# duyhominhnguyen/conan-fgw

Measured on AMD Instinct MI355X. Metric: molecules/s (K=5 conformers), higher is better.
Workload: dtype f32

## Files before the change

conan-fgw_amd/csrc/fgw_common.h:

```cpp
#pragma once
#include "common.h"

#ifdef CONAN_FGW_PROFILE
static __device__ long long g_fgw_prof[32];
#define FGW_PROF_ACCESSOR(name)                                                          \
    extern "C" int name(long long *out, int reset) {                                     \
        if (out && hipMemcpyFromSymbol(out, HIP_SYMBOL(g_fgw_prof), sizeof(long long) * 32) != hipSuccess) return -2; \
        if (reset) { long long z[32] = {0}; if (hipMemcpyToSymbol(HIP_SYMBOL(g_fgw_prof), z, sizeof(z)) != hipSuccess) return -2; } \
        return 0;                                                                        \
    }
static __device__ long long g_fgw_trace[2 + 6 * 8192];
#define FGW_PROF_TRACE_ACCESSOR(name)                                                    \
    extern "C" int name(long long *out, int reset) {                                     \
        if (out && hipMemcpyFromSymbol(out, HIP_SYMBOL(g_fgw_trace), sizeof(long long) * (2 + 6 * 8192)) != hipSuccess) return -2; \
        if (reset) { long long z[2] = {0, 0}; if (hipMemcpyToSymbol(HIP_SYMBOL(g_fgw_trace), z, sizeof(z)) != hipSuccess) return -2; } \
        return 0;                                                                        \
    }
#define FGW_PROF_TRACE(tag)                                                              \
    do {                                                                                 \
        if (threadIdx.x == 0) {                                                          \
            const unsigned long long i_ = atomicAdd(reinterpret_cast<unsigned long long *>(&g_fgw_trace[0]), 1ull); \
            if (i_ < 8192) {                                                             \
                long long *r_ = &g_fgw_trace[2 + 6 * i_];                                \
                r_[0] = (long long)blockIdx.x; r_[1] = (long long)(tag);                 \
// ... 214 lines not shown
                for (int u = 0; u < 4; ++u) a[u] = (double)xr[kb + u];
                if (WT) {
                    const TW *wr = W + (size_t)jc * pW + kb;
#pragma unroll
                    for (int u = 0; u < 4; ++u) b[u] = (double)wr[u];
                } else {
#pragma unroll
                    for (int u = 0; u < 4; ++u) b[u] = (double)W[(size_t)(kb + u) * pW + jc];
                }
            } else {
#pragma unroll
                for (int u = 0; u < 4; ++u) {
                    const int k = kb + u, kc = k < Kd ? k : Kd - 1;
                    const double av = (double)xr[kc], bv = (double)(WT ? W[(size_t)jc * pW + kc] : W[(size_t)kc * pW + jc]);
                    a[u] = k < Kd ? av : 0.0; b[u] = k < Kd ? bv : 0.0;
                }
            }
            acc = __builtin_amdgcn_mfma_f64_16x16x4f64(ra ? a[0] : 0.0, cb ? b[0] : 0.0, acc, 0, 0, 0);
            acc2 = __builtin_amdgcn_mfma_f64_16x16x4f64(ra ? a[1] : 0.0, cb ? b[1] : 0.0, acc2, 0, 0, 0);
            acc = __builtin_amdgcn_mfma_f64_16x16x4f64(ra ? a[2] : 0.0, cb ? b[2] : 0.0, acc, 0, 0, 0);
            acc2 = __builtin_amdgcn_mfma_f64_16x16x4f64(ra ? a[3] : 0.0, cb ? b[3] : 0.0, acc2, 0, 0, 0);
        }
#pragma unroll
        for (int q = 0; q < 4; ++q) {
            const int i = i0 + lk + 4 * q;
            if (i < M && cb) st(i, jb, acc[q] + acc2[q]);
        }
    }
}

template <int NT>
__device__ __forceinline__ void fgw_order_by_size(const FgwAdj &adj, int B, int K, int tid) {
    static_assert(NT >= 256, "one thread per size bin");
    __shared__ unsigned char nsz[4096];
    __shared__ int hist[256], base[256];
    if (B > 4096) return;
    for (int t = tid; t < 256; t += NT) hist[t] = 0;
    __syncthreads();
    for (int m = tid; m < B; m += NT) {
        const int n = min(max(adj.gptr[m * K + 1] - adj.gptr[m * K], 0), 255);
        nsz[m] = (unsigned char)n;
        atomicAdd(&hist[n], 1);
    }
    __syncthreads();
    if (tid == 0) {
        int run = 0;
        for (int v = 255; v >= 0; --v) { base[v] = run; run += hist[v]; }
    }
    __syncthreads();
    if (tid < 256 && hist[tid] > 0) {
        int pos = base[tid];
        for (int m = 0; m < B; ++m)
            if (nsz[m] == (unsigned char)tid) adj.order[pos++] = m;
    }
}

#ifndef CONAN_FGW_KT
#define CONAN_FGW_KT 2
#endif
template <int NW, bool WT, typename TX, typename TW, class FS, int KT = CONAN_FGW_KT>
__device__ __forceinline__ void mm_f64_glb22(int M, int Nn, int Kd, const TX *__restrict__ X, int pX, const TW *__restrict__ W, int pW, FS st,
                                             const int tid = threadIdx.x) {
    const int lane = tid & 63, wave = __builtin_amdgcn_readfirstlane(tid >> 6);
    const int Mq = (M + 15) >> 4, Nq = (Nn + 15) >> 4;
    const int li = lane & 15, lk = lane >> 4;
    const int Mb = Mq >> 1, Nb = Nq >> 1;
    const int nblk = Mb * Nb, nblk_used = (nblk / NW) * NW;
    auto load_a = [&](const TX *xr, int kb, int k0, double (&a)[KT]) {
        if (k0 + 4 * KT <= Kd) {
#pragma unroll
            for (int u = 0; u < KT; ++u) a[u] = (double)xr[kb + u];
        } else {
#pragma unroll
            for (int u = 0; u < KT; ++u) { const int k = kb + u; const double v = (double)xr[k < Kd ? k : Kd - 1]; a[u] = k < Kd ? v : 0.0; }
        }
    };
    auto load_b = [&](int jc, int kb, int k0, double (&b)[KT]) {
        if (k0 + 4 * KT <= Kd) {
#pragma unroll
            for (int u = 0; u < KT; ++u) b[u] = (double)(WT ? W[(size_t)jc * pW + kb + u] : W[(size_t)(kb + u) * pW + jc]);
        } else {
#pragma unroll
            for (int u = 0; u < KT; ++u) {
                const int k = kb + u, kc = k < Kd ? k : Kd - 1;
                const double v = (double)(WT ? W[(size_t)jc * pW + kc] : W[(size_t)kc * pW + jc]);
// ... 616 lines not shown
```

conan-fgw_amd/csrc/fgw_small.hip:

```cpp
#include "fgw_common.h"

#ifdef CONAN_FGW_PROFILE
FGW_PROF_ACCESSOR(conan_debug_fgw_prof)
FGW_PROF_TRACE_ACCESSOR(conan_debug_fgw_trace)
#endif

namespace {

constexpr int SK_SCRATCH_DOUBLES = 3 * 256 + 2 * 64;

template <int R, bool KL, bool SECOND = false>
__global__ void __launch_bounds__(FGW_THREADS, (SECOND || R > 9) ? 1 : 3) k_fgw_coupling_small(
    const float *__restrict__ Ys, const float *__restrict__ Cs, const float *__restrict__ ps, const float *__restrict__ pb,
    FgwDims D, conan_fgw_params prm, int outer, int y_zero, const double *__restrict__ Cw, const double *__restrict__ Yw,
    const int *__restrict__ active, float *__restrict__ Tw, int *__restrict__ info, fgw_part_t *__restrict__ Ypart,
    fgw_part_t *__restrict__ Cpart, const double *__restrict__ zvec, const double *__restrict__ yvec, const int *__restrict__ only, FgwAdj adj) {
    extern __shared__ __attribute__((aligned(16))) char smem[];
    auto solve = [&](const int cid) {
    const int b = cid / D.K, s = cid % D.K;
    if (!fgw_active(active, D.B, b, outer)) return;
    const int N = D.N, P = D.P, d = D.d;
    const int NN = N * N, NP = N * P;
    const int tid = threadIdx.x, lane = tid & 63, w = __builtin_amdgcn_readfirstlane(tid >> 6);
    const bool lane_ok = lane < N;
    FGW_PROF_DECL;

    double *Al = reinterpret_cast<double *>(smem);
    double *Gl = Al + NP;
    double *C1l = Gl + NP;
    double *Bl = C1l + NP;
    double *pq = Bl + NP;
    double *red = pq + 128;
    float *t_dummy = reinterpret_cast<float *>(red + 7);
    double *vec4 = red + 8;
    const bool alias = (size_t)NP >= SK_SCRATCH_DOUBLES;
    double *own = vec4 + 256;
    double *bufC = alias ? Al : own;
    double *bufK = bufC + 256;
    double *bufR = bufK + 256;
    double *fcp = bufR + 256;
    double *gcp = fcp + 64;
    float *Tl = reinterpret_cast<float *>(own + (alias ? 0 : SK_SCRATCH_DOUBLES));
// ... 11 lines not shown
    float *Tg = Tw + ((size_t)b * D.K + s) * NN;
    const double alpha = (double)prm.alpha, inv_eps = 1.0 / (double)prm.epsilon;

    constexpr int EPT = (16 * R * R + FGW_THREADS - 1) / FGW_THREADS;
    double c1v[EPT];
    float c2v[EPT], tv[EPT];
    const bool warm = outer > 0 && prm.warmstart;
#pragma unroll
    for (int u = 0; u < EPT; ++u) {
        const int t = tid + u * FGW_THREADS, tc = t < NN ? t : NN - 1;
        c1v[u] = C1[tc]; c2v[u] = C2[tc]; tv[u] = warm ? Tg[tc] : 0.f;
    }
    const double p_own = tid < N ? (pb ? (double)pb[(size_t)b * N + tid] : 1.0 / (double)N) : 1.0;
    const double q_own = tid < N ? (ps ? (double)ps[((size_t)b * D.K + s) * N + tid] : 1.0 / (double)N) : 1.0;
    double vec_own;
    {
        const int v = tid >> 6, i = tid & 63;
        const double *src = (v == 0 || v == 2) ? yvec + (size_t)b * 2 * N + (v == 0 ? N : 0) : zvec + ((size_t)b * D.K + s) * 2 * N + (v == 1 ? N : 0);
        vec_own = src[i < N ? i : N - 1];
        vec_own = i < N ? vec_own : 0.0;
    }
    const bool stage_yz = yz_lds && !y_zero;
    if (stage_yz) {
        const int Nd = N * d;
        for (int t0 = tid; t0 < Nd; t0 += 4 * FGW_THREADS) {
            double yv[4]; float zv[4];
#pragma unroll
            for (int u = 0; u < 4; ++u) { const int t = t0 + u * FGW_THREADS, tc = t < Nd ? t : Nd - 1; yv[u] = Y[tc]; zv[u] = Z[tc]; }
#pragma unroll
            for (int u = 0; u < 4; ++u) { const int t = t0 + u * FGW_THREADS; if (t < Nd) { Yl[t] = yv[u]; Zl[t] = zv[u]; } }
        }
    }
    if (tid < 64) { pq[tid] = p_own; pq[64 + tid] = q_own; }
    const bool massless = __syncthreads_or(tid < N && (p_own <= 0.0 || q_own <= 0.0)) != 0;
    vec4[tid] = vec_own;
#pragma unroll
    for (int u = 0; u < EPT; ++u) {
        const int t = tid + u * FGW_THREADS;
        if (t < NN) { const int i = t / N, j = t - i * N; C2l[i * P + j] = c2v[u]; if (!stage_yz) C1l[i * P + j] = c1v[u]; }
    }
    __syncthreads();
    FGW_PROF(0);
    const double qj = pq[64 + lane];
    const double pi_l = pq[lane];
#pragma unroll
    for (int u = 0; u < EPT; ++u) {
        const int t = tid + u * FGW_THREADS;
        if (t < NN) { const int i = t / N, j = t - i * N; Tl[i * P + j] = warm ? tv[u] : (float)(pq[i] * pq[64 + j]); }
    }
    const double *r1v = vec4, *r2v = vec4 + 64, *y2v = vec4 + 128, *z2v = vec4 + 192;
    double *Dl = stage_yz ? C1l : Al;
    if (!y_zero) {
        if (stage_yz)
            mm_lds<FGW_WAVES, true>(N, N, d, Yl, d, Zl, d, [&](int i, int j, double v) { Dl[i * P + j] = v; }, border_prepare(N, N));
        else
            mm_f64(N, N, d, [&](int i, int k) { return Y[(size_t)i * d + k]; }, [&](int k, int j) { return (double)Z[(size_t)j * d + k]; },
                   [&](int i, int j, double v) { Dl[i * P + j] = v; });
    }
    __syncthreads();
    FGW_PROF(1);
#pragma unroll
    for (int u = 0; u < EPT; ++u) {
        const int t = tid + u * FGW_THREADS;
        if (t < NN) {
            const int i = t / N, j = t - i * N;
            double m = -2.0 * (y_zero ? 0.0 : Dl[i * P + j]); m += y2v[i]; m += z2v[j];
            m = m > 0.0 ? m : 0.0;
// ... 138 lines not shown
                         xs[192 + lane] * exp_lse(m3 - M);
                    u_l = lane_ok ? loga - (log_acc(sm) + M) : 0.0;
                }
                uc[lane] = u_l;
                if (ii % 10 == 0) {
                    double cs = 0.0;
#pragma unroll
                    for (int r = 0; r < R; ++r) cs += exp_acc(mrA(r) + uc[w + 4 * r] + v_l);
                    __syncthreads();
                    xs[w * 64 + lane] = cs;
                    __syncthreads();
                    cs = ((xs[lane] + xs[64 + lane]) + xs[128 + lane]) + xs[192 + lane];
                    double df = lane_ok ? cs - qj : 0.0;
                    df = wave_sum_d(df * df);
                    if (sqrt(df) < (double)prm.stop_thr) { ++ii; break; }
                }
            }
#pragma unroll
            for (int r = 0; r < R; ++r) kA[r] = exp_acc(mrA(r) + uc[w + 4 * r] + v_l);
        }
        sk_total += ii;
        FGW_PROF(6);
        double e2 = 0.0;
#pragma unroll
        for (int r = 0; r < R; ++r) {
            const int i = wq + 4 * r;
            const bool ok = lane_ok && i < N;
            float *tp = ok ? &Tl[i * P + lq] : t_dummy;
            const float tn = (float)kA[r];
            const double df = ok ? (double)tn - (double)*tp : 0.0;
            e2 += df * df;
            *tp = tn;
        }
        if (cpt % 10 == 0) err = sqrt(block_sum_d(e2, red));
        else __syncthreads();
        ++cpt;
        FGW_PROF(7);
    }
    __syncthreads();
    for (int t = tid; t < NN; t += FGW_THREADS) { const int i = t / N, j = t - i * N; Tg[t] = Tl[i * P + j]; }
    if (tid == 0) { atomicAdd(&info[b * 4 + 1], cpt); atomicAdd(&info[b * 4 + 2], sk_total); }
    FGW_PROF(8);

    if (!prm.fixed_features && Ypart) {
        fgw_part_t *Yp = Ypart + ((size_t)b * D.K + s) * N * d;
        if (z_lds) {
            const int Nd = N * d;
            for (int t0 = tid; t0 < Nd; t0 += 4 * FGW_THREADS) {
                float zv[4];
#pragma unroll
                for (int u = 0; u < 4; ++u) { const int t = t0 + u * FGW_THREADS; zv[u] = Z[t < Nd ? t : Nd - 1]; }
#pragma unroll
                for (int u = 0; u < 4; ++u) { const int t = t0 + u * FGW_THREADS; if (t < Nd) Zl2[t] = zv[u]; }
            }
            __syncthreads();
            mm_lds<FGW_WAVES, false>(N, d, N, Tl, P, Zl2, d, [&](int i, int c, double v) { Yp[(size_t)i * d + c] = (fgw_part_t)v; }, border_prepare(N, d));
        } else {
            mm_f64(N, d, N, [&](int i, int k) { return (double)Tl[i * P + k]; }, [&](int k, int c) { return (double)Z[(size_t)k * d + c]; },
                   [&](int i, int c, double v) { Yp[(size_t)i * d + c] = (fgw_part_t)v; });
        }
    }
    FGW_PROF(9);
    if (!prm.fixed_structure) {
        fgw_part_t *Cp = Cpart + ((size_t)b * D.K + s) * NN;
        if constexpr (KL)
            mm_f64(N, N, N, [&](int i, int k) { return (double)Tl[i * P + k]; },
                   [&](int k, int j) { const double cv = (double)C2l[k * P + j]; return log(cv > 1e-15 ? cv : 1e-15); },
                   [&](int i, int j, double v) { Al[i * P + j] = v; }, bnn);
        else
            mm_lds<FGW_WAVES, false>(N, N, N, Tl, P, C2l, P, [&](int i, int j, double v) { Al[i * P + j] = v; }, bnn);
        __syncthreads();
        mm_lds<FGW_WAVES, true>(N, N, N, Al, P, Tl, P, [&](int i, int j, double v) { Cp[i * N + j] = (fgw_part_t)v; }, bnn);
    }
    FGW_PROF(10);
    FGW_PROF_FLUSH;
    };
    if constexpr (!SECOND) solve(blockIdx.x);
    else {
        const int total = D.B * D.K, base = (int)blockIdx.x * 64, l = (int)threadIdx.x & 63;
        unsigned long long m = __ballot(base + l < total && only[base + l < total ? base + l : 0] != 0);
        while (m) {
            const int k = __ffsll((long long)m) - 1;
            m &= m - 1;
            solve(base + k);
            __syncthreads();
        }
    }
}

template <int R> struct FastCfg {
    static constexpr int OCC = R <= 9 ? 5 : (R <= 12 ? 2 : 1);
};
inline int fast_tiles_per_wave(int N) {
    const int Mc = (N >> 4) << 4;
    const bool border = (N - Mc) * N + Mc * (N - Mc) <= FGW_WAVES * 32 && Mc > 0;
    const int q = border ? N >> 4 : (N + 15) >> 4;
    return (q * q + FGW_WAVES - 1) / FGW_WAVES;
}
constexpr int FAST_VEC_DOUBLES = 128 + 256;
constexpr int FAST_SK_DOUBLES = 2 * 256 + 2 * 64;

struct FastLds {
    int npa;
    size_t off_t, off_c2, off_red, off_vec, off_sk, off_rs, bytes;
    bool vec_alias, sk_alias;
};
template <typename C2T>
__host__ __device__ inline FastLds fast_lds(int N) {
    FastLds L;
    const int NP = N * fgw_pitch(N);
    L.npa = (NP + 1) & ~1;
    size_t o = (size_t)3 * L.npa * 8;
    L.off_t = o; o += ((size_t)NP * 4 + 15) & ~(size_t)15;
    L.off_c2 = o; o += ((size_t)NP * sizeof(C2T) + 15) & ~(size_t)15;
    L.off_red = o; o += 64;
    L.vec_alias = (size_t)NP * 4 >= FAST_VEC_DOUBLES * 8;
    L.sk_alias = L.npa >= FAST_SK_DOUBLES;
    L.off_vec = L.vec_alias ? L.off_t : o; if (!L.vec_alias) o += FAST_VEC_DOUBLES * 8;
    L.off_sk = L.sk_alias ? (size_t)L.npa * 8 : o; if (!L.sk_alias) o += FAST_SK_DOUBLES * 8;
    const bool rs_alias = (size_t)NP * sizeof(C2T) >= (size_t)4 * N * 8;
    L.off_rs = rs_alias ? L.off_c2 : o; if (!rs_alias) o += (size_t)4 * N * 8;
    L.bytes = o;
    return L;
}

template <int R, int MAXT, typename C2T>
__global__ void __launch_bounds__(FGW_THREADS, FastCfg<R>::OCC) k_fgw_coupling_fast(
    const float *__restrict__ Ys, const float *__restrict__ Cs, const float *__restrict__ ps, const float *__restrict__ pb,
    FgwDims D, conan_fgw_params prm, FastConst fc, int outer, int y_zero, const double *__restrict__ Cw, const double *__restrict__ Yw,
    const int *__restrict__ active, float *__restrict__ Tw, int *__restrict__ info, fgw_part_t *__restrict__ Ypart,
    fgw_part_t *__restrict__ Cpart, const double *__restrict__ zvec, const double *__restrict__ yvec, int *__restrict__ redo, FgwAdj adj) {
    extern __shared__ __attribute__((aligned(16))) char smem[];
    int cid = (gridDim.x & 7) == 0 ? xcd_contiguous_block((int)blockIdx.x, (int)gridDim.x) : (int)blockIdx.x;
    if (adj.order && (gridDim.x & 7) == 0) {
        const int x = (int)blockIdx.x & 7, pblk = (int)blockIdx.x >> 3;
        cid = adj.order[x + 8 * (pblk / D.K)] * D.K + pblk % D.K;
    }
    const int b = cid / D.K, s = cid % D.K;
    if (!fgw_active(active, D.B, b, outer)) return;
    const int N = D.N, P = D.P, d = D.d;
    const int NN = N * N;
    const int tid = threadIdx.x, lane = tid & 63, w = __builtin_amdgcn_readfirstlane(tid >> 6);
    FGW_PROF_DECL;

    const FastLds L = fast_lds<C2T>(N);
    double *C1l = reinterpret_cast<double *>(smem);
    double *AKl = C1l + L.npa;
    double *Bl = AKl + L.npa;
    float *Tl = reinterpret_cast<float *>(smem + L.off_t);
    C2T *C2l = reinterpret_cast<C2T *>(smem + L.off_c2);
    double *red = reinterpret_cast<double *>(smem + L.off_red);
    float *t_dummy = reinterpret_cast<float *>(red + 7);
    double *pq = reinterpret_cast<double *>(smem + L.off_vec);
    double *vec4 = pq + 128;
    double *bufC = reinterpret_cast<double *>(smem + L.off_sk);
    double *bufR = bufC + 256;
    double *fvP = bufR + 256;
    double *gvP = fvP + 64;
    double *Yl = AKl;
    float *Zl = reinterpret_cast<float *>(C1l);
// ... 52 lines not shown
        const double c_nb = C1[(size_t)nb_ * N + lc];
        const double cbb = __shfl(c_nb, nb_, 64);
        const double want = lane < nb_ ? c_nb : cbb;
        for (int r = nb_ + 1 + w; r < N; r += FGW_WAVES) ok = ok && (lane >= N || near(C1[(size_t)r * N + lc], want));
        ok = ok && (lane < nb_ || lane >= N || near(c_nb, cbb));
        const int mcol = N - nb_;
        for (int k = w; k < nb_; k += FGW_WAVES) {
            const double v = C1[(size_t)k * N + nb_ + (lane < mcol ? lane : 0)];
            ok = ok && near(v, __shfl(v, 0, 64));
        }
        return ok;
    };
    bool pad_ok = pad_try && ragged && N - nb >= 2 && nb >= 1;
    if (pad_ok) pad_ok = c1_block_ok(nb);
    if (stage_yz) {
        const int Nd = N * d;
        for (int t0 = tid; t0 < Nd; t0 += 4 * FGW_THREADS) {
            double yv[4]; float zv[4];
#pragma unroll
            for (int u = 0; u < 4; ++u) { const int t = t0 + u * FGW_THREADS, tc = t < Nd ? t : Nd - 1; yv[u] = Y[tc]; zv[u] = Z[tc]; }
#pragma unroll
            for (int u = 0; u < 4; ++u) { const int t = t0 + u * FGW_THREADS; if (t < Nd) { Yl[t] = yv[u]; Zl[t] = zv[u]; } }
        }
    }
    if (tid < 64) { pq[tid] = p_own; pq[64 + tid] = q_own; }
    vec4[tid] = vec_own;
    for_entries([&](int u, int o) { C2l[o] = (C2T)c2v[u]; if (!stage_yz) C1l[o] = c1v[u]; });
    if constexpr (sizeof(C2T) == 1) {
        if (ragged) {
            __syncthreads();
            adj_scatter_lds_bytes<FGW_THREADS>(adj, cid, N, P, reinterpret_cast<unsigned char *>(C2l), tid);
        }
    }
    __syncthreads();
    int n_real;
    {
        const bool nz = lane < N && C2l[lane] != (C2T)0;
        n_real = 1 + __popcll(__ballot(nz));
    }
    bool complete;
    {
        bool ok = true;
        int i = e_i0, j = e_j0;
#pragma unroll
        for (int u = 0; u < EPT; ++u) {
            if (tid + u * FGW_THREADS < NN) ok = ok && (C2l[i * P + j] == (C2T)((i != j && i < n_real && j < n_real) ? 1 : 0));
            j += e_dr; i += e_dq;
            if (j >= N) { j -= N; ++i; }
        }
        complete = __syncthreads_and(ok) != 0 && n_real >= 2;
    }
    double *rsum = reinterpret_cast<double *>(smem + L.off_rs);
    if (!ragged) {
        int mx = 1;
        int i = e_i0, j = e_j0;
#pragma unroll
        for (int u = 0; u < EPT; ++u) {
            if (tid + u * FGW_THREADS < NN && C2l[i * P + j] != (C2T)0) mx = max(mx, max(i, j) + 1);
            j += e_dr; i += e_dq;
            if (j >= N) { j -= N; ++i; }
        }
#pragma unroll
        for (int o = 32; o > 0; o >>= 1) mx = max(mx, __shfl_xor(mx, o, 64));
        int *ired = reinterpret_cast<int *>(red);
        if (lane == 0) ired[w] = mx;
        __syncthreads();
        nb = max(max(ired[0], ired[1]), max(ired[2], ired[3]));
        __syncthreads();
        pad_ok = pad_try && N - nb >= 2 && nb >= 1;
        if (pad_ok) pad_ok = c1_block_ok(nb);
    }
    int m_pad = 0;
    if (pad_try && N - nb >= 2 && nb >= 1) {
        auto nearf = [](double a, double b_) { return fabs(a - b_) <= 1e-9 * (fabs(b_) + 1e-30) || a == b_; };
        bool ok = pad_ok;
        for (int r = nb + 1 + w; r < N; r += FGW_WAVES)
            for (int c = lane; c < d; c += 64) {
                if (stage_yz) {
                    ok = ok && nearf((double)Zl[r * d + c], (double)Zl[nb * d + c]) && nearf(Yl[r * d + c], Yl[nb * d + c]);
                } else {
                    ok = ok && nearf((double)Z[(size_t)r * d + c], (double)Z[(size_t)nb * d + c]);
                    if (!y_zero) ok = ok && nearf(Y[(size_t)r * d + c], Y[(size_t)nb * d + c]);
                }
            }
        if (__syncthreads_and(ok) != 0) m_pad = N - nb;
    }
    const int Nx = m_pad ? nb + 1 : N;
    const double mult = m_pad ? (double)m_pad : 1.0;
    FGW_PROF(0);
    const double qj = pq[64 + lane] * ((m_pad && lane == nb) ? mult : 1.0);
    const double pi_l = pq[lane] * ((m_pad && lane == nb) ? mult : 1.0);
    const double *r1v = vec4, *r2v = vec4 + 64, *y2v = vec4 + 128, *z2v = vec4 + 192;
    auto base_of = [&](int i, int j, double dot) {
        double m = -2.0 * dot; m += y2v[i]; m += z2v[j];
        m = m > 0.0 ? m : 0.0;
        return fc.two_alpha * (r1v[i] + r2v[j]) + fc.one_m_alpha * m;
    };
    if (y_zero) {
        int i = e_i0, j = e_j0;
#pragma unroll
        for (int u = 0; u < EPT; ++u) {
            if (tid + u * FGW_THREADS < NN) Bl[i * P + j] = base_of(i, j, 0.0);
            j += e_dr; i += e_dq;
            if (j >= N) { j -= N; ++i; }
        }
    } else if (stage_yz) {
        mm_lds2<FGW_WAVES, MAXT, 0, true, true>(Nx, Nx, d, Yl, d, Zl, d, [&]() { load_c1_t(); __syncthreads(); },
                                                [&](int i, int j, double v) { Bl[i * P + j] = base_of(i, j, v); });
        for_entries([&](int u, int o) { C1l[o] = c1v[u]; });
    } else {
        mm_f64(Nx, Nx, d, [&](int i, int k) { return Y[(size_t)i * d + k]; }, [&](int k, int j) { return (double)Z[(size_t)j * d + k]; },
               [&](int i, int j, double v) { Bl[i * P + j] = base_of(i, j, v); });
    }
    __syncthreads();
    FGW_PROF(1);
    if (warm) {
        if (m_pad) {
            int i = e_i0, j = e_j0;
#pragma unroll
            for (int u = 0; u < EPT; ++u) {
                if (tid + u * FGW_THREADS < NN) Tl[i * P + j] = (float)((double)tv[u] * ((i == nb ? mult : 1.0) * (j == nb ? mult : 1.0)));
                j += e_dr; i += e_dq;
                if (j >= N) { j -= N; ++i; }
            }
        } else {
            for_entries([&](int u, int o) { Tl[o] = tv[u]; });
        }
    } else {
#pragma unroll
        for (int r = 0; r < R; ++r) {
            const int i = w + 4 * r;
            const double pi_r = (pb ? (double)pb[(size_t)b * N + (i < N ? i : N - 1)] : fc.inv_n) * ((m_pad && i == nb) ? mult : 1.0);
            if (i < Nx && lane < Nx) Tl[i * P + lane] = (float)(pi_r * qj);
        }
    }
    __syncthreads();
    FGW_PROF(2);

    int cpt = 0, sk_total = 0;
    double err = 1.0;
    bool bail = __syncthreads_or(tid < N && (p_own <= 0.0 || q_own <= 0.0)) != 0;
    while (!bail && err > fc.inner_tol && cpt < prm.max_iter) {
        int tq = tid, N = Nx, P = D.P;
        asm volatile("" : "+v"(tq), "+s"(N), "+s"(P));
        int nbq = m_pad ? nb : -1;
        asm volatile("" : "+s"(nbq));
        const int lq = tq & 63, wq = tq >> 6;
        const bool lq_ok = lq < N;
        mm_lds2<FGW_WAVES, 1, 0, false, false>(N, N, N, C1l, P, Tl, P, [] {}, [&](int i, int j, double v) { AKl[i * P + j] = v; }, tq);
        __syncthreads();
        FGW_PROF(3);
        int nr = n_real;
        asm volatile("" : "+s"(nr));
        if (complete) {
            {
                const int lc = lq_ok ? lq : N - 1;
                const double *ar = AKl + lc * P + wq;
                double p0 = 0.0, p1 = 0.0;
#pragma unroll
                for (int r = 0; r < R; ++r) {
                    const int q = wq + 4 * r;
                    if (q < nr) { if (r & 1) p1 += ar[4 * r]; else p0 += ar[4 * r]; }
                }
                if (lq_ok) rsum[wq * N + lq] = p0 + p1;
            }
            __syncthreads();
            {
                int i = tq / N, j = tq - i * N;
                const int dq = FGW_THREADS / N, dr = FGW_THREADS - dq * N;
                for (int t = tq; t < N * N; t += FGW_THREADS) {
                    const int o = i * P + j;
                    const double ai = ((rsum[i] + rsum[N + i]) + rsum[2 * N + i]) + rsum[3 * N + i];
                    const double v = j < nr ? ai - AKl[o] : 0.0;
                    const double x = fma(v, fc.four_alpha_inv_eps, (Bl[j * P + j] - Bl[o]) * fc.inv_eps);
// ... 38 lines not shown
        };
        int ii = 0;
        double f = 0.0, g = 0.0, colp = 0.0;
        bool have_colp = false;
        for (; ii < prm.num_iter_max; ++ii) {
            if (!have_colp) {
                double pc = 0.0;
                if (ii == 0) {
                    gvP[permL] = lq_ok ? (lq == nbq ? (double)m_pad : 1.0) : 0.0;
                }
                pc = dotR(kA, gw);
                *bufCw = pc;
                __syncthreads();
                colp = ((bufC[lq] + bufC[64 + lq]) + bufC[128 + lq]) + bufC[192 + lq];
            }
            have_colp = false;
            if (__any(lq_ok && !(colp > 1e-150 && colp < 1e150))) { bail = true; break; }
            f = lq_ok ? qj * rcp_pos(colp) : 0.0;
            fvP[permL] = f;
            *bufRw = dotR(kB, fw);
            __syncthreads();
            const double rs = ((bufR[lq] + bufR[64 + lq]) + bufR[128 + lq]) + bufR[192 + lq];
            if (__any(lq_ok && !(rs > 1e-150 && rs < 1e150))) { bail = true; break; }
            g = lq_ok ? pi_l * rcp_pos(rs) : 0.0;
            gvP[permL] = g;
            if (ii % 10 == 0) {
                *bufCw = dotR(kA, gw);
                __syncthreads();
                colp = ((bufC[lq] + bufC[64 + lq]) + bufC[128 + lq]) + bufC[192 + lq];
                have_colp = true;
                double df = lq_ok ? f * colp - qj : 0.0;
                df = df * df;
                if (lq == nbq) df /= (double)m_pad;
                df = wave_sum_d(df);
                if (sqrt(df) < fc.stop_thr) { ++ii; break; }
            }
        }
        if (bail) break;
        sk_total += ii;
        FGW_PROF(6);
        double e2 = 0.0;
        {
            float *trow = Tl + wq * P + lq;
#pragma unroll
            for (int r = 0; r < R; ++r) {
                const bool ok = lq_ok && wq + 4 * r < N;
                float *tp = ok ? trow + 4 * r * P : t_dummy;
                const float tn = (float)((gw[r] * kA[r]) * f);
                double df = ok ? (double)tn - (double)*tp : 0.0;
                df *= df;
                if (nbq >= 0) {
                    const double im = 1.0 / (double)m_pad;
                    df *= (lq == nbq ? im : 1.0) * (wq + 4 * r == nbq ? im : 1.0);
                }
                e2 += df;
                *tp = tn;
            }
        }
        if (cpt % 10 == 0) err = sqrt(block_sum_d(e2, red));
        else __syncthreads();
        ++cpt;
        FGW_PROF(7);
    }
    if (bail) {
        if (tid == 0) { redo[cid] = 1; atomicOr(&info[b * 4 + 3], 1); }
        return;
    }
    __syncthreads();
    {
        int te = tid;
        asm volatile("" : "+v"(te));
        int i = te / N, j = te - i * N;
        const int dq = FGW_THREADS / N, dr = FGW_THREADS - dq * N;
        if (m_pad) {
            const float im = (float)(1.0 / mult);
            for (int t = te; t < NN; t += FGW_THREADS) {
                Tg[t] = Tl[min(i, nb) * P + min(j, nb)] * ((i >= nb ? im : 1.0f) * (j >= nb ? im : 1.0f));
                j += dr; i += dq;
                if (j >= N) { j -= N; ++i; }
            }
        } else {
            for (int t = te; t < NN; t += FGW_THREADS) {
                Tg[t] = Tl[i * P + j];
                j += dr; i += dq;
                if (j >= N) { j -= N; ++i; }
            }
        }
    }
    if (tid == 0) { atomicAdd(&info[b * 4 + 1], cpt); atomicAdd(&info[b * 4 + 2], sk_total); redo[cid] = 0; if (m_pad) atomicOr(&info[b * 4 + 3], 2); }
    FGW_PROF(8);

    if (!prm.fixed_features && Ypart) {
        fgw_part_t *Yp = Ypart + ((size_t)b * D.K + s) * N * d;
        if (yz_lds) {
            const int Nd = N * d;
            for (int t0 = tid; t0 < Nd; t0 += 4 * FGW_THREADS) {
                float zv[4];
#pragma unroll
                for (int u = 0; u < 4; ++u) { const int t = t0 + u * FGW_THREADS; zv[u] = Z[t < Nd ? t : Nd - 1]; }
#pragma unroll
                for (int u = 0; u < 4; ++u) { const int t = t0 + u * FGW_THREADS; if (t < Nd) Zl[t] = zv[u]; }
            }
            __syncthreads();
            mm_lds2<FGW_WAVES, 1, 0, false, false>(N, d, N, Tl, P, Zl, d, [] {}, [&](int i, int c, double v) { Yp[(size_t)i * d + c] = (fgw_part_t)v; });
        } else {
            mm_f64(N, d, N, [&](int i, int k) { return (double)Tl[i * P + k]; }, [&](int k, int c) { return (double)Z[(size_t)k * d + c]; },
                   [&](int i, int c, double v) { Yp[(size_t)i * d + c] = (fgw_part_t)v; });
        }
    }
    FGW_PROF(9);
    if (!prm.fixed_structure) {
        fgw_part_t *Cp = Cpart + ((size_t)b * D.K + s) * NN;
        if (complete) {
            {
                const int lc = lane < Nx ? lane : Nx - 1;
                const float *tr = Tl + lc * P + w;
                double p0 = 0.0, p1 = 0.0;
#pragma unroll
                for (int r = 0; r < R; ++r) {
                    const int q = w + 4 * r;
                    if (q < n_real) { if (r & 1) p1 += (double)tr[4 * r]; else p0 += (double)tr[4 * r]; }
                }
                if (lane < Nx) rsum[w * N + lane] = p0 + p1;
            }
            __syncthreads();
            mm_lds2<FGW_WAVES, 1, 0, true, false>(Nx, Nx, n_real, Tl, P, Tl, P, [] {}, [&](int i, int j, double v) {
                const double ti = ((rsum[i] + rsum[N + i]) + rsum[2 * N + i]) + rsum[3 * N + i];
                const double tj = ((rsum[j] + rsum[N + j]) + rsum[2 * N + j]) + rsum[3 * N + j];
                if (m_pad) Bl[i * P + j] = ti * tj - v;
                else Cp[i * N + j] = (fgw_part_t)(ti * tj - v);
            });
        } else {
            mm_lds2<FGW_WAVES, 1, 0, false, false>(Nx, Nx, Nx, Tl, P, C2l, P, [] {}, [&](int i, int j, double v) { AKl[i * P + j] = v; });
            __syncthreads();
            mm_lds2<FGW_WAVES, 1, 0, true, false>(Nx, Nx, Nx, AKl, P, Tl, P, [] {}, [&](int i, int j, double v) {
                if (m_pad) Bl[i * P + j] = v;
                else Cp[i * N + j] = (fgw_part_t)v;
            });
        }
        if (m_pad) {
            __syncthreads();
            const double im = 1.0 / mult;
            int i = tid / N, j = tid - i * N;
            const int dq = FGW_THREADS / N, dr = FGW_THREADS - dq * N;
            for (int t = tid; t < NN; t += FGW_THREADS) {
                Cp[t] = (fgw_part_t)(Bl[min(i, nb) * P + min(j, nb)] * ((i >= nb ? im : 1.0) * (j >= nb ? im : 1.0)));
                j += dr; i += dq;
                if (j >= N) { j -= N; ++i; }
            }
        }
    }
    FGW_PROF(10);
    FGW_PROF_FLUSH;
    FGW_PROF_TRACE(Nx | (cpt << 8) | (sk_total << 20));
}

template <int NT>
__device__ __forceinline__ void molecule_vectors(const double *__restrict__ Y, const double *__restrict__ C, const float *__restrict__ p, int N,
                                                 int d, bool kl, double *__restrict__ out, int which = 2) {
    constexpr int LPI = NT / 64;
    const int i = (int)threadIdx.x / LPI, sub = (int)threadIdx.x % LPI;
    double y2 = 0.0, r1 = 0.0;
    if (i < N) {
        if (which != 1)
            for (int c = sub; c < d; c += LPI) { const double v = Y[(size_t)i * d + c]; y2 += v * v; }
        if (which != 0)
            for (int k = sub; k < N; k += LPI) {
                const double c1 = C[i * N + k], pk = p ? (double)p[k] : 1.0 / (double)N;
                r1 += (kl ? c1 * log(c1 + 1e-15) - c1 : c1 * c1) * pk;
            }
    }
#pragma unroll
    for (int o = 1; o < LPI; o <<= 1) { y2 += __shfl_xor(y2, o, 64); r1 += __shfl_xor(r1, o, 64); }
    if (i < N && sub == 0) { if (which != 1) out[i] = y2; if (which != 0) out[N + i] = r1; }
}

__global__ void __launch_bounds__(256) k_fgw_small_vectors(const float *__restrict__ Ys, const float *__restrict__ Cs, const float *__restrict__ ps,
                                                           const float *__restrict__ pb, FgwDims D, int kl, double *__restrict__ Cw,
                                                           double *__restrict__ Yw, double *__restrict__ zvec, double *__restrict__ yvec,
                                                           const float *__restrict__ init_C, const float *__restrict__ init_Y, int max_iter,
                                                           int *__restrict__ active, int *__restrict__ info, float *__restrict__ errs,
                                                           float *__restrict__ Yout, float *__restrict__ Cout, FgwAdj adj) {
    const int b = blockIdx.x / D.K, s = blockIdx.x % D.K;
    const int N = D.N, d = D.d;
    __shared__ __attribute__((aligned(16))) unsigned char cm[64 * 65 + 16];
    const int Pm = D.P;
    if (adj.rowptr) {
        for (int t = threadIdx.x; t < (64 * 65 + 16) / 4; t += 256) reinterpret_cast<unsigned *>(cm)[t] = 0u;
        __syncthreads();
        adj_scatter_lds_bytes<256>(adj, (int)blockIdx.x, N, Pm, cm, (int)threadIdx.x);
        __syncthreads();
    }
    if (s == 0) {
        const int NN = N * N, Nd = N * d;
        const float *c0 = init_C ? init_C + (size_t)b * NN : Cs + (size_t)b * D.K * NN;
        for (int t = threadIdx.x; t < NN; t += 256) {
            const float cv = (!init_C && adj.rowptr) ? (float)cm[(t / N) * Pm + (t % N)] : c0[t];
            Cw[(size_t)b * NN + t] = (double)cv; Cout[(size_t)b * NN + t] = cv;
        }
        for (int t = threadIdx.x; t < Nd; t += 256) {
            const float y = init_Y ? init_Y[(size_t)b * Nd + t] : 0.f;
            Yw[(size_t)b * Nd + t] = (double)y; Yout[(size_t)b * Nd + t] = y;
        }
        if (threadIdx.x == 0) { fgw_active_init(active, D.B, b); info[b * 4 + 0] = 0; info[b * 4 + 1] = 0; info[b * 4 + 2] = 0; info[b * 4 + 3] = 0; }
        for (int t = threadIdx.x; t < 2 * max_iter; t += 256) errs[(size_t)b * 2 * max_iter + t] = __builtin_nanf("");
        __syncthreads();
    }
    const float *Z = Ys + ((size_t)b * D.K + s) * N * d;
    const float *C2 = Cs + ((size_t)b * D.K + s) * N * N;
    const float *q = ps ? ps + ((size_t)b * D.K + s) * N : nullptr;
    const int j = (int)threadIdx.x >> 2, sub = (int)threadIdx.x & 3;
    double z2 = 0.0, r2 = 0.0;
    if (j < N) {
        for (int c = sub; c < d; c += 4) { const double v = (double)Z[(size_t)j * d + c]; z2 += v * v; }
        for (int k = sub; k < N; k += 4) {
            const double c2 = adj.rowptr ? (double)cm[j * Pm + k] : (double)C2[j * N + k], qk = q ? (double)q[k] : 1.0 / (double)N;
            r2 += qk * (kl ? c2 : c2 * c2);
        }
    }
    z2 += __shfl_xor(z2, 1, 64); z2 += __shfl_xor(z2, 2, 64);
    r2 += __shfl_xor(r2, 1, 64); r2 += __shfl_xor(r2, 2, 64);
    double *zo = zvec + ((size_t)b * D.K + s) * 2 * N;
    if (j < N && sub == 0) { zo[j] = z2; zo[N + j] = r2; }
    if (s == 0)
        molecule_vectors<256>(Yw + (size_t)b * N * d, Cw + (size_t)b * N * N, pb ? pb + (size_t)b * N : nullptr, N, d, kl != 0, yvec + (size_t)b * 2 * N);
    if (adj.order && blockIdx.x == gridDim.x - 1) fgw_order_by_size<256>(adj, D.B, D.K, (int)threadIdx.x);
}

constexpr int UPD_THREADS = 512;
template <bool Y_FROM_T>
__global__ void __launch_bounds__(UPD_THREADS) k_fgw_update_parts(
    const float *__restrict__ pb, const float *__restrict__ lambdas, FgwDims D, conan_fgw_params prm, int outer,
    const fgw_part_t *__restrict__ Ypart, const fgw_part_t *__restrict__ Cpart, double *__restrict__ Cw, double *__restrict__ Yw,
    int *__restrict__ active, int *__restrict__ info, float *__restrict__ errs, float *__restrict__ Yout, float *__restrict__ Cout,
    double *__restrict__ yvec, const float *__restrict__ Tw, const float *__restrict__ Ys, int chunk) {
    __shared__ double red[UPD_THREADS / 64 + 1];
    extern __shared__ __attribute__((aligned(16))) char usmem[];
    const int part = (int)blockIdx.x >= D.B ? 1 : 0;
    const int b = (int)blockIdx.x - part * D.B;
    const int N = D.N, d = D.d, K = D.K, NN = N * N, Nd = N * d;
    const int tid = threadIdx.x;
    int *flag_out = active + (outer & 1) * 2 * D.B + part * D.B + b;
    if (!fgw_active(active, D.B, b, outer)) {
        if (tid == 0) *flag_out = 0;
        return;
    }
    constexpr int U = 4;
    double e2 = 0.0;
    if (part == 0) {
        if (!prm.fixed_features) {
            double *Yb = Yw + (size_t)b * Nd;
            if constexpr (Y_FROM_T) {
                float *Tl = reinterpret_cast<float *>(usmem), *Zl = Tl + (size_t)chunk * NN;
                const int lane = tid & 63, wave = __builtin_amdgcn_readfirstlane(tid >> 6), li = lane & 15, lk = lane >> 4;
                const int Mq = (N + 15) >> 4, Nq = (d + 15) >> 4;
                constexpr int NWU = UPD_THREADS / 64, TW = 2;
                for (int t0 = 0; t0 < Mq * Nq; t0 += NWU * TW) {
                    int ti0[TW], tj0[TW], tic[TW], tjc[TW];
                    bool mine[TW];
// ... 113 lines not shown
                }
            }
        }
    }
    const double err = sqrt(block_sum_d<UPD_THREADS / 64>(e2, red));
    if (yvec) molecule_vectors<UPD_THREADS>(Yw + (size_t)b * Nd, Cw + (size_t)b * NN, pb ? pb + (size_t)b * N : nullptr, N, d, prm.loss_fun != 0,
                                            yvec + (size_t)b * 2 * N, part);
    if (tid == 0) {
        errs[((size_t)b * 2 + part) * prm.max_iter + outer] = (float)err;
        info[b * 4 + 0] = outer + 1;
        *flag_out = err > (double)prm.tol ? 1 : 0;
    }
}

inline size_t small_lds(int N, int d) {
    const size_t NP = (size_t)N * fgw_pitch(N);
    (void)d; return NP * 8 * 4 + (256 + 128 + 8 + (NP >= (size_t)SK_SCRATCH_DOUBLES ? 0 : SK_SCRATCH_DOUBLES)) * 8 + NP * 4 * 2;
}

}

bool conan_fgw_small_supported(int N, int d) { return N <= 64 && small_lds(N, d) <= 160 * 1024; }

size_t conan_fgw_part_offset(int B, int K, int N, int d) {
    return (((size_t)B * K * N * d + (size_t)B * K * N * N) * sizeof(fgw_part_t) + 15) & ~(size_t)15;
}
size_t conan_fgw_small_part_bytes(int B, int K, int N, int d) {
    return conan_fgw_part_offset(B, K, N, d) + ((size_t)B * K * 2 * N + (size_t)B * 2 * N) * 8 + (size_t)B * K * 4 + 512;
}

void conan_fgw_small_prepare(const float *Ys, const float *Cs, const float *ps, const float *pb, FgwDims D, conan_fgw_params prm,
                             double *Cw, double *Yw, double *zvec, double *yvec, const float *init_C, const float *init_Y, int *active, int *info,
                             float *errs, float *Yout, float *Cout, FgwAdj adj, hipStream_t s) {
    k_fgw_small_vectors<<<D.B * D.K, 256, 0, s>>>(Ys, Cs, ps, pb, D, prm.loss_fun, Cw, Yw, zvec, yvec, init_C, init_Y, prm.max_iter, active, info,
                                                 errs, Yout, Cout, adj);
}

template <int R, int MAXT, typename C2T>
static void launch_fast_t(const float *Ys, const float *Cs, const float *ps, const float *pb, FgwDims D, conan_fgw_params prm, int outer, int y_zero,
                        const double *Cw, const double *Yw, const int *active, float *Tw, int *info, fgw_part_t *Ypart, fgw_part_t *Cpart,
                        const double *zvec, const double *yvec, int *redo, FgwAdj adj, hipStream_t s) {
    const size_t lds = fast_lds<C2T>(D.N).bytes;
    if (lds > 64 * 1024)
        (void)hipFuncSetAttribute(reinterpret_cast<const void *>(&k_fgw_coupling_fast<R, MAXT, C2T>), hipFuncAttributeMaxDynamicSharedMemorySize,
                                  (int)lds);
    const FastConst fc = fast_const(prm, D.N);
    k_fgw_coupling_fast<R, MAXT, C2T><<<D.B * D.K, FGW_THREADS, lds, s>>>(Ys, Cs, ps, pb, D, prm, fc, outer, y_zero, Cw, Yw, active, Tw, info, Ypart,
                                                                          Cpart, zvec, yvec, redo, adj);
}
template <int R, typename C2T>
static void launch_fast(const float *Ys, const float *Cs, const float *ps, const float *pb, FgwDims D, conan_fgw_params prm, int outer, int y_zero,
                        const double *Cw, const double *Yw, const int *active, float *Tw, int *info, fgw_part_t *Ypart, fgw_part_t *Cpart,
                        const double *zvec, const double *yvec, int *redo, FgwAdj adj, hipStream_t s) {
    const int tpw = fast_tiles_per_wave(D.N);
#define ARGS Ys, Cs, ps, pb, D, prm, outer, y_zero, Cw, Yw, active, Tw, info, Ypart, Cpart, zvec, yvec, redo, adj, s
    if constexpr (R <= 6) launch_fast_t<R, 1, C2T>(ARGS);
    else if constexpr (R <= 12) { if (tpw <= 1) launch_fast_t<R, 1, C2T>(ARGS); else launch_fast_t<R, 3, C2T>(ARGS); }
    else { if (tpw <= 1) launch_fast_t<R, 1, C2T>(ARGS); else if (tpw <= 3) launch_fast_t<R, 3, C2T>(ARGS); else launch_fast_t<R, 4, C2T>(ARGS); }
#undef ARGS
}

bool conan_fgw_fast_supported(int N, int d, int small_int) {
    if (N > 64 || N < 4) return false;
    const size_t lds = small_int ? fast_lds<unsigned char>(N).bytes : fast_lds<float>(N).bytes;
    return lds <= 160 * 1024 && d >= 1;
}

// ... 74 lines not shown
```

Measured before the change: 115,100.

## Scalarize uniform values, lower fast-kernel occupancy hint, and front-load size ordering block

Wraps block-uniform reductions and flags in readfirstlane so the compiler keeps them in scalar registers. It also lowers the occupancy target for MAXT>1 fast kernels and caches 1/m_pad in shared memory. The size-ordering pass moves from the last block of the vectors kernel to a dedicated first block, and it now computes prefix positions per thread with vectorized LDS reads instead of a serial scan plus an extra barrier. Together these aim to cut VGPR pressure, barriers and tail latency, but they change register allocation and the order of several statements.

```diff
diff --git a/conan-fgw_amd/csrc/fgw_common.h b/conan-fgw_amd/csrc/fgw_common.h
--- a/conan-fgw_amd/csrc/fgw_common.h
+++ b/conan-fgw_amd/csrc/fgw_common.h
@@ -270,8 +270,8 @@
 template <int NT>
 __device__ __forceinline__ void fgw_order_by_size(const FgwAdj &adj, int B, int K, int tid) {
     static_assert(NT >= 256, "one thread per size bin");
-    __shared__ unsigned char nsz[4096];
-    __shared__ int hist[256], base[256];
+    __shared__ __attribute__((aligned(16))) unsigned char nsz[4096];
+    __shared__ __attribute__((aligned(16))) int hist[256];
     if (B > 4096) return;
     for (int t = tid; t < 256; t += NT) hist[t] = 0;
     __syncthreads();
@@ -281,14 +281,23 @@
         atomicAdd(&hist[n], 1);
     }
     __syncthreads();
-    if (tid == 0) {
-        int run = 0;
-        for (int v = 255; v >= 0; --v) { base[v] = run; run += hist[v]; }
-    }
-    __syncthreads();
     if (tid < 256 && hist[tid] > 0) {
-        int pos = base[tid];
-        for (int m = 0; m < B; ++m)
+        int pos = 0;
+        for (int v4 = tid >> 2; v4 < 64; ++v4) {
+            const int4 h = reinterpret_cast<const int4 *>(hist)[v4];
+            const int v = 4 * v4;
+            pos += (v > tid ? h.x : 0) + (v + 1 > tid ? h.y : 0) + (v + 2 > tid ? h.z : 0) + (v + 3 > tid ? h.w : 0);
+        }
+        const unsigned me = (unsigned)tid;
+        int m = 0;
+        for (; m + 16 <= B; m += 16) {
+            const uint4 q = *reinterpret_cast<const uint4 *>(nsz + m);
+            const unsigned wds[4] = {q.x, q.y, q.z, q.w};
+#pragma unroll
+            for (int u = 0; u < 16; ++u)
+                if (((wds[u >> 2] >> (8 * (u & 3))) & 255u) == me) adj.order[pos++] = m + u;
+        }
+        for (; m < B; ++m)
             if (nsz[m] == (unsigned char)tid) adj.order[pos++] = m;
     }
 }
diff --git a/conan-fgw_amd/csrc/fgw_small.hip b/conan-fgw_amd/csrc/fgw_small.hip
--- a/conan-fgw_amd/csrc/fgw_small.hip
+++ b/conan-fgw_amd/csrc/fgw_small.hip
@@ -8,6 +8,12 @@
 namespace {
 
 constexpr int SK_SCRATCH_DOUBLES = 3 * 256 + 2 * 64;
+
+__device__ __forceinline__ int uni(int v) { return __builtin_amdgcn_readfirstlane(v); }
+__device__ __forceinline__ bool uni(bool v) { return __builtin_amdgcn_readfirstlane((int)v) != 0; }
+__device__ __forceinline__ double uni(double v) {
+    return __hiloint2double(__builtin_amdgcn_readfirstlane(__double2hiint(v)), __builtin_amdgcn_readfirstlane(__double2loint(v)));
+}
 
 template <int R, bool KL, bool SECOND = false>
 __global__ void __launch_bounds__(FGW_THREADS, (SECOND || R > 9) ? 1 : 3) k_fgw_coupling_small(
@@ -85,7 +91,7 @@
         }
     }
     if (tid < 64) { pq[tid] = p_own; pq[64 + tid] = q_own; }
-    const bool massless = __syncthreads_or(tid < N && (p_own <= 0.0 || q_own <= 0.0)) != 0;
+    const bool massless = uni(__syncthreads_or(tid < N && (p_own <= 0.0 || q_own <= 0.0)) != 0);
     vec4[tid] = vec_own;
 #pragma unroll
     for (int u = 0; u < EPT; ++u) {
@@ -290,7 +296,7 @@
             e2 += df * df;
             *tp = tn;
         }
-        if (cpt % 10 == 0) err = sqrt(block_sum_d(e2, red));
+        if (cpt % 10 == 0) err = uni(sqrt(block_sum_d(e2, red)));
         else __syncthreads();
         ++cpt;
         FGW_PROF(7);
@@ -346,8 +352,8 @@
     }
 }
 
-template <int R> struct FastCfg {
-    static constexpr int OCC = R <= 9 ? 5 : (R <= 12 ? 2 : 1);
+template <int R, int MAXT> struct FastCfg {
+    static constexpr int OCC = R <= 9 ? (MAXT == 1 ? 5 : 4) : (R <= 12 ? 2 : 1);
 };
 inline int fast_tiles_per_wave(int N) {
     const int Mc = (N >> 4) << 4;
@@ -383,7 +389,7 @@
 }
 
 template <int R, int MAXT, typename C2T>
-__global__ void __launch_bounds__(FGW_THREADS, FastCfg<R>::OCC) k_fgw_coupling_fast(
+__global__ void __launch_bounds__(FGW_THREADS, (FastCfg<R, MAXT>::OCC)) k_fgw_coupling_fast(
     const float *__restrict__ Ys, const float *__restrict__ Cs, const float *__restrict__ ps, const float *__restrict__ pb,
     FgwDims D, conan_fgw_params prm, FastConst fc, int outer, int y_zero, const double *__restrict__ Cw, const double *__restrict__ Yw,
     const int *__restrict__ active, float *__restrict__ Tw, int *__restrict__ info, fgw_part_t *__restrict__ Ypart,
@@ -502,7 +508,7 @@
             adj_scatter_lds_bytes<FGW_THREADS>(adj, cid, N, P, reinterpret_cast<unsigned char *>(C2l), tid);
         }
     }
-    __syncthreads();
+    bool bail = uni(__syncthreads_or(tid < N && (p_own <= 0.0 || q_own <= 0.0)) != 0);
     int n_real;
     {
         const bool nz = lane < N && C2l[lane] != (C2T)0;
@@ -518,7 +524,7 @@
             j += e_dr; i += e_dq;
             if (j >= N) { j -= N; ++i; }
         }
-        complete = __syncthreads_and(ok) != 0 && n_real >= 2;
+        complete = uni(__syncthreads_and(ok) != 0) && n_real >= 2;
     }
     double *rsum = reinterpret_cast<double *>(smem + L.off_rs);
     if (!ragged) {
@@ -535,7 +541,7 @@
         int *ired = reinterpret_cast<int *>(red);
         if (lane == 0) ired[w] = mx;
         __syncthreads();
-        nb = max(max(ired[0], ired[1]), max(ired[2], ired[3]));
+        nb = uni(max(max(ired[0], ired[1]), max(ired[2], ired[3])));
         __syncthreads();
         pad_ok = pad_try && N - nb >= 2 && nb >= 1;
         if (pad_ok) pad_ok = c1_block_ok(nb);
@@ -553,13 +559,12 @@
                     if (!y_zero) ok = ok && nearf(Y[(size_t)r * d + c], Y[(size_t)nb * d + c]);
                 }
             }
-        if (__syncthreads_and(ok) != 0) m_pad = N - nb;
+        if (uni(__syncthreads_and(ok) != 0)) m_pad = N - nb;
     }
     const int Nx = m_pad ? nb + 1 : N;
     const double mult = m_pad ? (double)m_pad : 1.0;
+    if (tid == 0) red[6] = 1.0 / (double)m_pad;
     FGW_PROF(0);
-    const double qj = pq[64 + lane] * ((m_pad && lane == nb) ? mult : 1.0);
-    const double pi_l = pq[lane] * ((m_pad && lane == nb) ? mult : 1.0);
     const double *r1v = vec4, *r2v = vec4 + 64, *y2v = vec4 + 128, *z2v = vec4 + 192;
     auto base_of = [&](int i, int j, double dot) {
         double m = -2.0 * dot; m += y2v[i]; m += z2v[j];
@@ -582,6 +587,8 @@
         mm_f64(Nx, Nx, d, [&](int i, int k) { return Y[(size_t)i * d + k]; }, [&](int k, int j) { return (double)Z[(size_t)j * d + k]; },
                [&](int i, int j, double v) { Bl[i * P + j] = base_of(i, j, v); });
     }
+    const double qj = pq[64 + lane] * ((m_pad && lane == nb) ? mult : 1.0);
+    const double pi_l = pq[lane] * ((m_pad && lane == nb) ? mult : 1.0);
     __syncthreads();
     FGW_PROF(1);
     if (warm) {
@@ -609,7 +616,6 @@
 
     int cpt = 0, sk_total = 0;
     double err = 1.0;
-    bool bail = __syncthreads_or(tid < N && (p_own <= 0.0 || q_own <= 0.0)) != 0;
     while (!bail && err > fc.inner_tol && cpt < prm.max_iter) {
         int tq = tid, N = Nx, P = D.P;
         asm volatile("" : "+v"(tq), "+s"(N), "+s"(P));
@@ -714,7 +720,7 @@
                 double df = lq_ok ? f * colp - qj : 0.0;
                 df = df * df;
                 if (lq == nbq) df /= (double)m_pad;
-                df = wave_sum_d(df);
+                df = uni(wave_sum_d(df));
                 if (sqrt(df) < fc.stop_thr) { ++ii; break; }
             }
         }
@@ -732,14 +738,14 @@
                 double df = ok ? (double)tn - (double)*tp : 0.0;
                 df *= df;
                 if (nbq >= 0) {
-                    const double im = 1.0 / (double)m_pad;
+                    const double im = red[6];
                     df *= (lq == nbq ? im : 1.0) * (wq + 4 * r == nbq ? im : 1.0);
                 }
                 e2 += df;
                 *tp = tn;
             }
         }
-        if (cpt % 10 == 0) err = sqrt(block_sum_d(e2, red));
+        if (cpt % 10 == 0) err = uni(sqrt(block_sum_d(e2, red)));
         else __syncthreads();
         ++cpt;
         FGW_PROF(7);
@@ -755,7 +761,7 @@
         int i = te / N, j = te - i * N;
         const int dq = FGW_THREADS / N, dr = FGW_THREADS - dq * N;
         if (m_pad) {
-            const float im = (float)(1.0 / mult);
+            const float im = (float)red[6];
             for (int t = te; t < NN; t += FGW_THREADS) {
                 Tg[t] = Tl[min(i, nb) * P + min(j, nb)] * ((i >= nb ? im : 1.0f) * (j >= nb ? im : 1.0f));
                 j += dr; i += dq;
@@ -772,11 +778,14 @@
     if (tid == 0) { atomicAdd(&info[b * 4 + 1], cpt); atomicAdd(&info[b * 4 + 2], sk_total); redo[cid] = 0; if (m_pad) atomicOr(&info[b * 4 + 3], 2); }
     FGW_PROF(8);
 
+    int tz = tid;
+    asm volatile("" : "+v"(tz));
+    const int lz = tz & 63, wz = __builtin_amdgcn_readfirstlane(tz >> 6);
     if (!prm.fixed_features && Ypart) {
         fgw_part_t *Yp = Ypart + ((size_t)b * D.K + s) * N * d;
         if (yz_lds) {
             const int Nd = N * d;
-            for (int t0 = tid; t0 < Nd; t0 += 4 * FGW_THREADS) {
+            for (int t0 = tz; t0 < Nd; t0 += 4 * FGW_THREADS) {
                 float zv[4];
 #pragma unroll
                 for (int u = 0; u < 4; ++u) { const int t = t0 + u * FGW_THREADS; zv[u] = Z[t < Nd ? t : Nd - 1]; }
@@ -784,7 +793,7 @@
                 for (int u = 0; u < 4; ++u) { const int t = t0 + u * FGW_THREADS; if (t < Nd) Zl[t] = zv[u]; }
             }
             __syncthreads();
-            mm_lds2<FGW_WAVES, 1, 0, false, false>(N, d, N, Tl, P, Zl, d, [] {}, [&](int i, int c, double v) { Yp[(size_t)i * d + c] = (fgw_part_t)v; });
+            mm_lds2<FGW_WAVES, 1, 0, false, false>(N, d, N, Tl, P, Zl, d, [] {}, [&](int i, int c, double v) { Yp[(size_t)i * d + c] = (fgw_part_t)v; }, tz);
         } else {
             mm_f64(N, d, N, [&](int i, int k) { return (double)Tl[i * P + k]; }, [&](int k, int c) { return (double)Z[(size_t)k * d + c]; },
                    [&](int i, int c, double v) { Yp[(size_t)i * d + c] = (fgw_part_t)v; });
@@ -795,15 +804,15 @@
         fgw_part_t *Cp = Cpart + ((size_t)b * D.K + s) * NN;
         if (complete) {
             {
-                const int lc = lane < Nx ? lane : Nx - 1;
-                const float *tr = Tl + lc * P + w;
+                const int lc = lz < Nx ? lz : Nx - 1;
+                const float *tr = Tl + lc * P + wz;
                 double p0 = 0.0, p1 = 0.0;
 #pragma unroll
                 for (int r = 0; r < R; ++r) {
-                    const int q = w + 4 * r;
+                    const int q = wz + 4 * r;
                     if (q < n_real) { if (r & 1) p1 += (double)tr[4 * r]; else p0 += (double)tr[4 * r]; }
                 }
-                if (lane < Nx) rsum[w * N + lane] = p0 + p1;
+                if (lz < Nx) rsum[wz * N + lz] = p0 + p1;
             }
             __syncthreads();
             mm_lds2<FGW_WAVES, 1, 0, true, false>(Nx, Nx, n_real, Tl, P, Tl, P, [] {}, [&](int i, int j, double v) {
@@ -811,21 +820,21 @@
                 const double tj = ((rsum[j] + rsum[N + j]) + rsum[2 * N + j]) + rsum[3 * N + j];
                 if (m_pad) Bl[i * P + j] = ti * tj - v;
                 else Cp[i * N + j] = (fgw_part_t)(ti * tj - v);
-            });
+            }, tz);
         } else {
-            mm_lds2<FGW_WAVES, 1, 0, false, false>(Nx, Nx, Nx, Tl, P, C2l, P, [] {}, [&](int i, int j, double v) { AKl[i * P + j] = v; });
+            mm_lds2<FGW_WAVES, 1, 0, false, false>(Nx, Nx, Nx, Tl, P, C2l, P, [] {}, [&](int i, int j, double v) { AKl[i * P + j] = v; }, tz);
             __syncthreads();
             mm_lds2<FGW_WAVES, 1, 0, true, false>(Nx, Nx, Nx, AKl, P, Tl, P, [] {}, [&](int i, int j, double v) {
                 if (m_pad) Bl[i * P + j] = v;
                 else Cp[i * N + j] = (fgw_part_t)v;
-            });
+            }, tz);
         }
         if (m_pad) {
             __syncthreads();
-            const double im = 1.0 / mult;
-            int i = tid / N, j = tid - i * N;
+            const double im = red[6];
+            int i = tz / N, j = tz - i * N;
             const int dq = FGW_THREADS / N, dr = FGW_THREADS - dq * N;
-            for (int t = tid; t < NN; t += FGW_THREADS) {
+            for (int t = tz; t < NN; t += FGW_THREADS) {
                 Cp[t] = (fgw_part_t)(Bl[min(i, nb) * P + min(j, nb)] * ((i >= nb ? im : 1.0) * (j >= nb ? im : 1.0)));
                 j += dr; i += dq;
                 if (j >= N) { j -= N; ++i; }
@@ -863,14 +872,16 @@
                                                            const float *__restrict__ init_C, const float *__restrict__ init_Y, int max_iter,
                                                            int *__restrict__ active, int *__restrict__ info, float *__restrict__ errs,
                                                            float *__restrict__ Yout, float *__restrict__ Cout, FgwAdj adj) {
-    const int b = blockIdx.x / D.K, s = blockIdx.x % D.K;
+    if (adj.order && blockIdx.x == 0) { fgw_order_by_size<256>(adj, D.B, D.K, (int)threadIdx.x); return; }
+    const int blk = (int)blockIdx.x - (adj.order ? 1 : 0);
+    const int b = blk / D.K, s = blk % D.K;
     const int N = D.N, d = D.d;
     __shared__ __attribute__((aligned(16))) unsigned char cm[64 * 65 + 16];
     const int Pm = D.P;
     if (adj.rowptr) {
         for (int t = threadIdx.x; t < (64 * 65 + 16) / 4; t += 256) reinterpret_cast<unsigned *>(cm)[t] = 0u;
         __syncthreads();
-        adj_scatter_lds_bytes<256>(adj, (int)blockIdx.x, N, Pm, cm, (int)threadIdx.x);
+        adj_scatter_lds_bytes<256>(adj, blk, N, Pm, cm, (int)threadIdx.x);
         __syncthreads();
     }
     if (s == 0) {
@@ -906,7 +917,6 @@
     if (j < N && sub == 0) { zo[j] = z2; zo[N + j] = r2; }
     if (s == 0)
         molecule_vectors<256>(Yw + (size_t)b * N * d, Cw + (size_t)b * N * N, pb ? pb + (size_t)b * N : nullptr, N, d, kl != 0, yvec + (size_t)b * 2 * N);
-    if (adj.order && blockIdx.x == gridDim.x - 1) fgw_order_by_size<256>(adj, D.B, D.K, (int)threadIdx.x);
 }
 
 constexpr int UPD_THREADS = 512;
@@ -1086,7 +1096,7 @@
 void conan_fgw_small_prepare(const float *Ys, const float *Cs, const float *ps, const float *pb, FgwDims D, conan_fgw_params prm,
                              double *Cw, double *Yw, double *zvec, double *yvec, const float *init_C, const float *init_Y, int *active, int *info,
                              float *errs, float *Yout, float *Cout, FgwAdj adj, hipStream_t s) {
-    k_fgw_small_vectors<<<D.B * D.K, 256, 0, s>>>(Ys, Cs, ps, pb, D, prm.loss_fun, Cw, Yw, zvec, yvec, init_C, init_Y, prm.max_iter, active, info,
+    k_fgw_small_vectors<<<D.B * D.K + (adj.order ? 1 : 0), 256, 0, s>>>(Ys, Cs, ps, pb, D, prm.loss_fun, Cw, Yw, zvec, yvec, init_C, init_Y, prm.max_iter, active, info,
                                                  errs, Yout, Cout, adj);
 }
 
```

Result: no change. 115,300, median of 3 (+0.2%).
